# zhangmozhe/Deep-Exemplar-based-Video-Colorization

Hardware: AMD Instinct MI355X
Metric: colorized frames/sec/GPU at 216x384; correlation HBM GB/s vs roofline (higher is better)
Workload: dtype f32

## Files before the change

deep-exemplar-based-video-colorization_amd/dvc_amd/_lib.py:

```python
import ctypes
import os

_HERE = os.path.dirname(os.path.abspath(__file__))
DEBUG_BUILD = os.environ.get("DVC_DEBUG_LIB", "0") == "1"
LIB_PATH = os.path.join(_HERE, "libdvc_hip_debug.so" if DEBUG_BUILD else "libdvc_hip.so")
ABI_VERSION = 20

c_float_p = ctypes.c_void_p
c_i32 = ctypes.c_int32
c_i64 = ctypes.c_int64


class DvcConvDesc(ctypes.Structure):
    _fields_ = [
        ("N", c_i32), ("Cin", c_i32), ("H", c_i32), ("W", c_i32),
        ("Cout", c_i32), ("ksize", c_i32), ("stride", c_i32), ("dil", c_i32),
        ("pad", c_i32), ("pad_mode", c_i32), ("in_up", c_i32), ("in_sub", c_i32),
        ("act", c_i32), ("act_slope", ctypes.c_float), ("in_prelu", c_i32), ("cfg", c_i32), ("split_k", c_i32),
        ("x_batch_stride", c_i64), ("y_batch_stride", c_i64), ("res_batch_stride", c_i64),
        ("flags", c_i32), ("w_batch_stride", c_i64),
    ]


class DvcConvGroupItem(ctypes.Structure):
    _fields_ = [
        ("d", DvcConvDesc), ("x", ctypes.c_void_p), ("u_packed", ctypes.c_void_p), ("bias", ctypes.c_void_p),
        ("act_slope_ptr", ctypes.c_void_p), ("residual", ctypes.c_void_p), ("y", ctypes.c_void_p),
        ("workspace", ctypes.c_void_p), ("workspace_bytes", ctypes.c_size_t),
    ]


class DvcInstNormItem(ctypes.Structure):
    _fields_ = [
        ("x", ctypes.c_void_p), ("S", c_i32), ("bias", ctypes.c_void_p), ("act", c_i32), ("act_slope", ctypes.c_float),
        ("act_slope_ptr", ctypes.c_void_p), ("residual", ctypes.c_void_p), ("slope_ptr", ctypes.c_void_p),
        ("chan_scale", ctypes.c_void_p), ("eps", ctypes.c_float),
        ("N", c_i32), ("C", c_i32), ("H", c_i32), ("W", c_i32), ("up", c_i32), ("sub", c_i32), ("rpad", c_i32),
        ("x_batch_stride", c_i64), ("res_batch_stride", c_i64), ("y_batch_stride", c_i64), ("y", ctypes.c_void_p),
    ]


_VP = ctypes.c_void_p
SIGNATURES = {
    "dvc_abi_version": (ctypes.c_int, []),
    "dvc_last_error": (ctypes.c_char_p, []),
    "dvc_conv2d_out_hw": (ctypes.c_int, [ctypes.POINTER(DvcConvDesc), ctypes.POINTER(c_i32), ctypes.POINTER(c_i32)]),
    "dvc_conv2d": (ctypes.c_int, [ctypes.POINTER(DvcConvDesc), _VP, _VP, _VP, _VP, _VP, _VP, _VP, _VP, _VP, _VP,
                                  ctypes.c_size_t, _VP]),
    "dvc_winograd_weight_floats": (ctypes.c_size_t, [c_i32, c_i32]),
    "dvc_winograd_pack_weight": (ctypes.c_int, [_VP, c_i32, c_i32, _VP, _VP]),
    "dvc_conv2d_winograd_split": (ctypes.c_int, [ctypes.POINTER(DvcConvDesc), ctypes.c_size_t, ctypes.POINTER(c_i32),
                                                ctypes.POINTER(c_i32)]),
    "dvc_conv2d_winograd": (ctypes.c_int, [ctypes.POINTER(DvcConvDesc), _VP, _VP, _VP, _VP, _VP, _VP, _VP,
                                           ctypes.c_size_t, _VP]),
    "dvc_conv2d_winograd_pool": (ctypes.c_int, [ctypes.POINTER(DvcConvDesc), _VP, _VP, _VP, _VP, _VP, _VP, c_i64, _VP,
                                                ctypes.c_size_t, _VP]),
    "dvc_conv2d_winograd_dual": (ctypes.c_int, [ctypes.POINTER(DvcConvDesc), ctypes.POINTER(DvcConvDesc), _VP, _VP, _VP, _VP, _VP,
                                                _VP, _VP, ctypes.c_size_t, _VP]),
    "dvc_conv2d_ws_eligible": (ctypes.c_int, [ctypes.POINTER(DvcConvDesc)]),
    "dvc_conv2d_ws_pack_weight": (ctypes.c_int, [_VP, c_i32, c_i32, _VP, _VP]),
    "dvc_conv2d_ws": (ctypes.c_int, [ctypes.POINTER(DvcConvDesc), _VP, _VP, _VP, _VP, _VP, _VP]),
    "dvc_conv2d_winograd_group": (ctypes.c_int, [ctypes.POINTER(DvcConvGroupItem), c_i32, _VP]),
    "dvc_instnorm_apply_group": (ctypes.c_int, [ctypes.POINTER(DvcInstNormItem), c_i32, _VP]),
    "dvc_conv1x1_small": (ctypes.c_int, [_VP, _VP, _VP, c_i32, c_i32, c_i32, c_i32, c_i32, _VP, _VP]),
    "dvc_instnorm_stats": (ctypes.c_int, [_VP, c_i32, c_i32, c_i32, c_i64, ctypes.c_float, _VP, _VP, _VP, _VP]),
    "dvc_affine_act": (ctypes.c_int, [_VP, _VP, _VP, _VP, _VP, c_i32, c_i32, c_i32, c_i32, c_i32, c_i32,
                                      c_i64, c_i64, c_i64, _VP, _VP]),
    "dvc_instnorm_apply": (ctypes.c_int, [_VP, _VP, _VP, _VP, ctypes.c_float, c_i32, c_i32, c_i32, c_i32, c_i32,
                                          c_i32, c_i32, c_i64, c_i64, c_i64, _VP, _VP, _VP, _VP, c_i32, _VP, _VP]),
    "dvc_cx_prepare": (ctypes.c_int, [_VP, _VP, c_i32, c_i32, c_i32, c_i32, ctypes.c_float, _VP, _VP, _VP, _VP]),
    "dvc_cx_rows": (ctypes.c_int, [_VP, c_i32, c_i64, c_i64, c_i32, c_i32, ctypes.c_float, _VP, _VP, _VP, _VP, _VP, _VP]),
    "dvc_cx_colmax": (ctypes.c_int, [_VP, c_i32, c_i64, c_i64, _VP, _VP, c_i32, c_i32, c_i32, ctypes.c_float, _VP, _VP, _VP]),
    "dvc_cx_finish": (ctypes.c_int, [_VP, c_i32, c_i32, _VP, _VP, _VP]),
    "dvc_cx_rows_tq": (ctypes.c_int, [_VP, c_i32, c_i64, c_i64, c_i64, _VP, _VP, _VP, c_i32, c_i32, c_i32, ctypes.c_float, _VP, _VP,
                                      _VP]),
    "dvc_cx_ds": (ctypes.c_int, [_VP, c_i32, c_i64, c_i64, c_i64, _VP, _VP, _VP, _VP, _VP, _VP, _VP, _VP, _VP, ctypes.c_float, c_i32,
                                 c_i32, c_i32, c_i32, c_i32, ctypes.c_float, _VP, _VP, _VP]),
    "dvc_cx_normalize_bwd": (ctypes.c_int, [_VP, _VP, _VP, c_i32, c_i32, c_i32, ctypes.c_float, _VP, _VP]),
    "dvc_instnorm_apply_partials": (ctypes.c_int, [_VP, c_i32, _VP, c_i32, ctypes.c_float, _VP, _VP, _VP, _VP, ctypes.c_float,
                                                   c_i32, c_i32, c_i32, c_i32, c_i32, c_i32, c_i32, c_i64, c_i64, _VP, _VP, _VP,
                                                   _VP, c_i32, _VP, _VP]),
    "dvc_maxpool2x2": (ctypes.c_int, [_VP, c_i32, c_i32, c_i32, _VP, _VP]),
    "dvc_avgpool2x2": (ctypes.c_int, [_VP, c_i32, c_i32, c_i32, _VP, _VP]),
    "dvc_avgpool4x4": (ctypes.c_int, [_VP, c_i32, c_i32, c_i32, _VP, _VP]),
    "dvc_upsample_nearest": (ctypes.c_int, [_VP, c_i32, c_i32, c_i32, c_i32, _VP, _VP]),
    "dvc_channel_l2norm": (ctypes.c_int, [_VP, c_i32, c_i32, c_i32, ctypes.c_float, _VP, _VP]),
    "dvc_channel_l2norm_multi": (ctypes.c_int, [_VP, _VP, _VP, _VP, c_i32, c_i32, ctypes.c_float, _VP]),
    "dvc_gray2rgb": (ctypes.c_int, [_VP, c_i32, c_i32, c_i64, _VP, _VP]),
    "dvc_lab2rgb": (ctypes.c_int, [_VP, c_i32, c_i32, ctypes.c_float, _VP, _VP]),
    "dvc_pack_color_input": (ctypes.c_int, [_VP, c_i64, _VP, _VP, _VP, c_i64, _VP, c_i64, c_i32, c_i32, _VP, _VP]),
    "dvc_upsample_bilinear2x": (ctypes.c_int, [_VP, c_i32, c_i32, c_i32, ctypes.c_float, _VP, _VP]),
    "dvc_lum_guide_u8": (ctypes.c_int, [_VP, c_i64, _VP, _VP]),
    "dvc_fgs_workspace_bytes": (ctypes.c_size_t, [c_i32, c_i32, c_i32, c_i32, c_i32]),
    "dvc_fgs_filter": (ctypes.c_int, [_VP, _VP, c_i32, c_i32, c_i32, c_i32, ctypes.c_float, ctypes.c_float, c_i32,
                                      ctypes.c_float, _VP, _VP, ctypes.c_size_t, _VP]),
    "dvc_lab2rgb_u8": (ctypes.c_int, [_VP, _VP, c_i32, c_i32, _VP, _VP]),
    "dvc_rgb8_to_lab": (ctypes.c_int, [_VP, c_i32, c_i32, _VP, _VP]),
    "dvc_center_pad_workspace_bytes": (ctypes.c_size_t, [c_i32, c_i32]),
    "dvc_center_pad_is_fused": (ctypes.c_int, [c_i32, c_i32, c_i32, c_i32]),
    "dvc_center_pad": (ctypes.c_int, [_VP, c_i32, c_i32, c_i32, c_i32, _VP, _VP, ctypes.c_size_t, _VP]),
    "dvc_corr_prepare": (ctypes.c_int, [_VP, c_i32, c_i32, c_i32, ctypes.c_float, _VP, _VP, _VP]),
    "dvc_corr_workspace_bytes": (ctypes.c_size_t, [c_i32, c_i32]),
    "dvc_corr_fwd": (ctypes.c_int, [_VP, _VP, _VP, ctypes.c_float, ctypes.c_float, c_i32, c_i32, c_i32, c_i32,
                                    _VP, _VP, _VP, _VP, _VP, _VP, ctypes.c_size_t, _VP]),
    "dvc_corr_merge_pack": (ctypes.c_int, [_VP, ctypes.c_size_t, ctypes.c_float, c_i32, c_i32, _VP, _VP, _VP, _VP, _VP, _VP, _VP]),
    "dvc_corr_prepare_bf16": (ctypes.c_int, [_VP, c_i32, c_i32, c_i32, ctypes.c_float, _VP, _VP, _VP, _VP]),
    "dvc_corr_bf16_workspace_bytes": (ctypes.c_size_t, [c_i32, c_i32]),
    "dvc_corr_fwd_bf16": (ctypes.c_int, [_VP, _VP, _VP, _VP, _VP, ctypes.c_float, c_i32, c_i32, c_i32, c_i32,
                                         _VP, _VP, _VP, _VP, _VP, _VP, ctypes.c_size_t, _VP]),
    "dvc_corr_softmax_bwd": (ctypes.c_int, [_VP, _VP, _VP, _VP, _VP, _VP, _VP, ctypes.c_float, ctypes.c_float, c_i32, c_i32, c_i32, c_i64, c_i32,
                                            _VP, _VP, _VP, _VP]),
    "dvc_nlwa_workspace_bytes": (ctypes.c_size_t, [c_i32, c_i32, c_i32, c_i32, c_i32]),
    "dvc_nlwa_fwd": (ctypes.c_int, [_VP, c_i32, c_i32, c_i32, _VP, c_i32, c_i32, c_i32, c_i32, c_i32, c_i32, ctypes.c_float,
                                    ctypes.c_float, ctypes.c_float, ctypes.c_float, c_i32, ctypes.c_float, _VP, _VP,
                                    ctypes.c_size_t, _VP]),
    "dvc_lwa_fwd": (ctypes.c_int, [_VP, c_i32, c_i32, c_i32, _VP, c_i32, c_i32, c_i32, c_i32, c_i32, ctypes.c_float,
                                   ctypes.c_float, ctypes.c_float, c_i32, ctypes.c_float, _VP, _VP]),
    "dvc_lwa_bwd": (ctypes.c_int, [_VP, c_i32, c_i32, c_i32, _VP, c_i32, c_i32, c_i32, c_i32, c_i32, ctypes.c_float,
                                   ctypes.c_float, ctypes.c_float, c_i32, ctypes.c_float, _VP, _VP, _VP, _VP, _VP]),
    "dvc_flow_warp_bwd_workspace_bytes": (ctypes.c_size_t, [c_i32, c_i32, c_i32, c_i32]),
    "dvc_flow_warp_fwd": (ctypes.c_int, [_VP, _VP, c_i32, c_i32, c_i32, c_i32, c_i32, _VP, _VP]),
    "dvc_flow_warp_bwd": (ctypes.c_int, [_VP, _VP, _VP, c_i32, c_i32, c_i32, c_i32, c_i32, _VP, _VP, _VP, ctypes.c_size_t, _VP]),
    "dvc_bgemm_workspace_bytes": (ctypes.c_size_t, [c_i32, c_i32, c_i32, c_i32]),
    "dvc_bgemm": (ctypes.c_int, [_VP, _VP, _VP, c_i32, c_i32, c_i32, c_i32, c_i64, c_i64, c_i64, c_i64, c_i64, c_i64, c_i64, c_i64,
                                 c_i32, _VP]),
    "dvc_bgemm_splitk": (ctypes.c_int, [_VP, _VP, _VP, c_i32, c_i32, c_i32, c_i32, c_i64, c_i64, c_i64, c_i64, c_i64, c_i64, c_i64,
                                        c_i64, c_i32, _VP, ctypes.c_size_t, _VP]),
    "dvc_vgg_act_bwd": (ctypes.c_int, [_VP, _VP, _VP, c_i64, _VP, _VP]),
    "dvc_vgg_pool_act_bwd": (ctypes.c_int, [_VP, _VP, _VP, _VP, c_i32, c_i32, c_i32, c_i32, _VP, _VP]),
    "dvc_vgg_conv1_bwd": (ctypes.c_int, [_VP, _VP, c_i32, c_i32, c_i32, c_i32, _VP, _VP]),
    "dvc_lab2rgb_bwd": (ctypes.c_int, [_VP, c_i32, c_i32, ctypes.c_float, _VP, _VP, _VP]),
# ... 69 lines not shown
```

deep-exemplar-based-video-colorization_amd/dvc_amd/nets.py:

```python
import torch
import torch.nn as nn
from torch.autograd.function import once_differentiable

from . import arch, ops

_VGG_MEAN_BGR = (0.40760392, 0.45795686, 0.48501961)


_pack_epoch = 0


def pack_epoch():
    return _pack_epoch


class _PackCache:

    def __init__(self):
        self._d = {}

    def get(self, key, param, fn):
        params = param if isinstance(param, tuple) else (param,)
        tag = tuple((p.data_ptr(), _version_of(p), str(p.device)) for p in params)
        param = params[0]
# ... 329 lines not shown
        self.phi = nn.Conv2d(self.in_channels, self.inter_channels, kernel_size=1, stride=1, padding=0)
        self._cache = _PackCache()
        self.corr_precision = "fp32"

    def _use_bf16(self, temperature, WTA_scale_weight):
        return self.corr_precision == "bf16" and float(temperature) <= 1e-4 and WTA_scale_weight == 1

    def _pk(self, key, conv):
        return self._cache.get(key, conv.weight, ops.pack_conv_weight)

    def _conv3(self, key, conv, x, **kw):
        return ops.conv3x3(x, conv.weight, _packs(self._cache, key, conv.weight), conv.bias.detach(), layer="warp." + key, **kw)

    def prepare(self):
        for hd in arch.WARP_HEAD_PLAN:
            for ci in (hd.conv_a, hd.conv_b):
                _prepack(self._cache, f"{hd.name}.{ci}", getattr(self, hd.name)[ci])
        for b in range(arch.WARP_NUM_RESBLOCKS):
            _prepack(self._cache, f"layer.{b}.conv1", self.layer[b].conv1)
            _prepack(self._cache, f"layer.{b}.conv2", self.layer[b].conv2)
        self._pk("theta", self.theta)
        self._pk("phi", self.phi)

    def features(self, r2, r3, r4, r5):
        return self._trunk(self._heads(r2, r3, r4, r5))

    def _heads(self, r2, r3, r4, r5):
        feats = [r2, r3, r4, r5]
        N = r2.shape[0]
        h, w, rpad5 = arch.warp_trunk_geometry([x.shape[2:] for x in feats])
        trunk = torch.empty((N, arch.WARP_TRUNK_CH, h, w), device=r2.device, dtype=torch.float32)
        bs = arch.WARP_TRUNK_CH * h * w
        heads = arch.WARP_HEAD_PLAN
        seqs = [getattr(self, hd.name) for hd in heads]

        def conv_item(hd, ci, x, **kw):
            key, conv = f"{hd.name}.{ci}", seqs[hd.index][ci]
            return dict(x=x, weight=conv.weight, packs=_packs(self._cache, key, conv.weight), bias=conv.bias.detach(),
                        layer="warp." + key, pad_mode=ops.PAD_REFLECT, **kw)

        t1 = ops.conv3x3_group([conv_item(hd, hd.conv_a, feats[hd.index], defer_reduce=hd.stride_b == 1) for hd in heads])
        normed = ops.instnorm_apply_group([dict(x=t, out=None if isinstance(t, ops.ConvPartials) else t,
                                                slope_t=seq[hd.prelu_a].weight.detach()) for hd, seq, t in zip(heads, seqs, t1)])
        t2 = [None] * len(heads)
        for hd, seq in zip(heads, seqs):
            if hd.stride_b != 1:
                cb = seq[hd.conv_b]
                t2[hd.index] = ops.conv2d(normed[hd.index], self._pk(f"{hd.name}.{hd.conv_b}", cb), cb.bias.detach(),
                                          stride=hd.stride_b, pad_mode=ops.PAD_REFLECT, in_up=2 if hd.up_mid else 1)
        plain = [hd for hd in heads if hd.stride_b == 1]
        second = ops.conv3x3_group([conv_item(hd, hd.conv_b, normed[hd.index], in_up=2 if hd.up_mid else 1, defer_reduce=True)
                                    for hd in plain])
        for hd, t in zip(plain, second):
            t2[hd.index] = t
        ops.instnorm_apply_group([dict(x=t, slope_t=seq[hd.prelu_b].weight.detach(), up=2 if hd.up_out else 1,
                                       rpad=rpad5 if hd.name == "layer5_1" else 0,
                                       out=trunk[:, hd.index * arch.WARP_FEATURE_CH:(hd.index + 1) * arch.WARP_FEATURE_CH],
                                       out_batch_stride=bs) for hd, seq, t in zip(heads, seqs, t2)])
        return trunk

    def _trunk(self, x, saved=None):
        for b in range(arch.WARP_NUM_RESBLOCKS):
            blk = self.layer[b]
            a = blk.prelu.weight.detach()
            if saved is not None:
                planes = x.shape[0] * x.shape[1]
                r1, r2 = (torch.empty(planes, device=x.device, dtype=torch.float32) for _ in range(2))
                t = self._conv3(f"layer.{b}.conv1", blk.conv1, x, pad_mode=ops.PAD_REFLECT)
                n1 = ops.instnorm_apply(t, out=t, scale_out=r1)
                p1 = ops.warp_prelu_fwd(n1, a)
                t = self._conv3(f"layer.{b}.conv2", blk.conv2, p1, pad_mode=ops.PAD_REFLECT)
                n2 = ops.instnorm_apply(t, out=t, scale_out=r2)
                saved.update({f"x{b}": x, f"n1.{b}": n1, f"rstd1.{b}": r1, f"p1.{b}": p1, f"n2.{b}": n2, f"rstd2.{b}": r2})
                x = ops.warp_prelu_fwd(n2, a, skip=x)
                continue
            t = self._conv3(f"layer.{b}.conv1", blk.conv1, x, pad_mode=ops.PAD_REFLECT, defer_reduce=True)
            t = _norm_in_place(t, slope_t=a)
            t = self._conv3(f"layer.{b}.conv2", blk.conv2, t, pad_mode=ops.PAD_REFLECT, defer_reduce=True)
            x = _norm_in_place(t, residual=x, slope_t=a)
        return x

    def project(self, which, feats, bf16=False, saved=None):
        conv = getattr(self, which)
        t = ops.conv2d(feats, self._pk(which, conv), conv.bias.detach(), ksize=1, pad=0)
        if saved is not None:
            assert not bf16
            out, mean = ops.corr_prepare_with_mean(t)
            saved["t." + which], saved["mean." + which] = t, mean
            return out
        return ops.corr_prepare_bf16(t) if bf16 else ops.corr_prepare(t)

    _HEADS = tuple(arch.WARP_HEAD_ORDER)

    def _trunk_named_parameters(self):
        return [(n, p) for n, p in self.named_parameters() if n.split(".")[0] in ("layer", "theta", "phi")]

    def _head_named_parameters(self):
        return [(n, p) for n, p in self.named_parameters() if n.split(".")[0] in self._HEADS]

    def _takes_training_path(self):
        return self.training and torch.is_grad_enabled() and any(p.requires_grad for _, p in self._trunk_named_parameters())

    def _check_training_call(self, exemplar_cache, return_taps, defer_merge, detach_flag):
        unfrozen = [n for n, p in self._head_named_parameters() if p.requires_grad]
        if unfrozen:
            raise NotImplementedError(
                f"WarpNet: the training path gives the gradients of the residual trunk and the theta / phi projections only "
                f"(layer.*, theta.*, phi.*); {len(unfrozen)} head parameters require grad ({unfrozen[0]}, ...); freeze the heads: "
                "`for head in (net.layer2_1, net.layer3_1, net.layer4_1, net.layer5_1): "
                "[p.requires_grad_(False) for p in head.parameters()]`")
        for flag, what in ((exemplar_cache is not None, "exemplar_cache"), (return_taps, "return_taps"), (defer_merge, "defer_merge"),
                           (detach_flag, "detach_flag=True")):
            if flag:
                raise NotImplementedError(f"WarpNet: `{what}` is not supported on the training path (training mode, grad mode on, "
                                          "a trunk / projection parameter requiring grad); call under torch.no_grad() or .eval()")

    def _forward_with_grad(self, ins, temperature, WTA_scale_weight):
        B_lab_map, A2, A3, A4, A5, B2, B3, B4, B5 = ins
        fh, fw = int(B_lab_map.shape[2] / 4), int(B_lab_map.shape[3] / 4)
        _check_trainable(self._trunk_named_parameters(), "WarpNet")
        with torch.no_grad():
            trunkA = self._heads(A2, A3, A4, A5)
            trunkB = self._heads(B2, B3, B4, B5)
            blab = ops.avgpool4x4(B_lab_map)
        if (trunkA.shape[2], trunkA.shape[3]) != (fh, fw):
            raise RuntimeError(f"shape '[{B_lab_map.shape[0]}, 1, {fh}, {fw}]' is invalid for feature map "
                               f"of size {tuple(trunkA.shape[2:])}")
        return self._train_from_trunks(trunkA, trunkB, blab, temperature, WTA_scale_weight)

    def _train_from_trunks(self, trunkA, trunkB, blab, temperature, WTA_scale_weight=1):
        from .corr_autograd import fused_correlation
        N, _, fh, fw = trunkA.shape
        named = self._trunk_named_parameters()
        theta, phi = _WarpTrain.apply(trunkA, trunkB, self, tuple(n for n, _ in named), *(p for _, p in named))
        y, sim, _ = fused_correlation(theta, phi, blab.view(N, 3, -1), float(temperature), fh, fw, WTA_scale_weight)
        return _Up4.apply(y), _Up4.apply(sim)

    def _trunk_forward_saving(self, trunkA, trunkB, saved):
        N = trunkA.shape[0]
        F = self._trunk(torch.cat((trunkA, trunkB), 0), saved=saved)
        saved["F"] = F
        return self.project("theta", F[:N], saved=saved), self.project("phi", F[N:], saved=saved)

    def _trunk_backward(self, t, g_theta, g_phi, need, need_trunk_input_grad=False):
        grads = {}
        F = t["F"]
        M, C, h, w = F.shape
        N = M // 2
        dF = torch.empty_like(F)
        need_blocks = need_trunk_input_grad or any(n.startswith("layer.") for n in need)
        for which, g, sl in (("theta", g_theta, slice(0, N)), ("phi", g_phi, slice(N, M))):
            conv = getattr(self, which)
            dt = ops.warp_cn_bwd(t["t." + which], t["mean." + which], g.contiguous())
            if _wants(need, which):
                _put_wb(grads, need, which, *ops.warp_k1_wgrad(dt, F[sl]))
            if need_blocks:
                wt = self._cache.get("warp_bwd." + which, conv.weight,
                                     lambda w: ops.pack_conv_weight(w.detach().transpose(0, 1).contiguous()))
                ops.conv2d(dt.view(N, -1, h, w), wt, None, ksize=1, pad=0, out=dF[sl])
        if not need_blocks:
            return None, None, grads
        g = dF
        for b in reversed(range(arch.WARP_NUM_RESBLOCKS)):
            blk = self.layer[b]
            a = blk.prelu.weight.detach()
            c1, c2 = f"layer.{b}.conv1", f"layer.{b}.conv2"
            sp = torch.empty((2, M * C), device=F.device, dtype=torch.float64)
            dz, du, _ = ops.warp_norm_prelu_bwd(g, t[f"n2.{b}"], t[f"rstd2.{b}"], a, skip=t[f"x{b}"], slope_part=sp[0])
            if _wants(need, c2):
                _put_wb(grads, need, c2, *ops.cvn_wgrad(dz, ops.warp_reflect_pad(t[f"p1.{b}"])))
            wt, packs = _bwd_filters(self._cache, "warp_bwd." + c2, blk.conv2.weight, vgg_bwd_weight)
            gp = ops.conv3x3(dz, wt, packs, None, layer="warp_bwd." + c2)
            g = ops.warp_fold(gp)
            del gp, dz
            dz, _, _ = ops.warp_norm_prelu_bwd(g, t[f"n1.{b}"], t[f"rstd1.{b}"], a, slope_part=sp[1])
            if _wants(need, c1):
                _put_wb(grads, need, c1, *ops.cvn_wgrad(dz, ops.warp_reflect_pad(t[f"x{b}"])))
            if f"layer.{b}.prelu.weight" in need:
                grads[f"layer.{b}.prelu.weight"] = ops.warp_slope_sum(sp)
            if b == 0 and not need_trunk_input_grad:
                return None, None, grads
            wt, packs = _bwd_filters(self._cache, "warp_bwd." + c1, blk.conv1.weight, vgg_bwd_weight)
            gp = ops.conv3x3(dz, wt, packs, None, layer="warp_bwd." + c1)
            g = ops.warp_fold(gp, skip=du)
            del gp, dz, du
        return g[:N], g[N:], grads

    def _memo_exemplar_side(self, key_tensors, regime, compute):
        mode = ops.exemplar_memo_mode()
        if mode == "off":
            return compute()
        versions = [_version_of(t) for t in key_tensors]
        pfp = tuple((p.data_ptr(), _version_of(p)) for p in self.parameters())
        if any(v is None for v in versions) or any(v is None for _, v in pfp):
            return compute()
        fp = (pfp, regime, ops.conv_algo(), ops.direct_layers(), ops.fuse_reduce(), ops.autotune_enabled(),
              ops.batch_plan_enabled(), ops.group_heads(), ops.ws_conv_enabled())
        memo = getattr(self, "_exemplar_memo", None)
        if (memo is not None and memo[1] == fp and len(memo[0]) == len(key_tensors)
                and all(a is b and va == vb for (a, va), b, vb in zip(memo[0], key_tensors, versions))):
            if mode != "verify":
                return memo[2]
            fresh = compute()
            if _same_tensors(fresh, memo[2]):
                return memo[2]
            import warnings
            warnings.warn("DVC_EXEMPLAR_MEMO=verify: the memoised exemplar side differs from a recomputation although no key "
                          "tensor or WarpNet parameter changed identity or version — something wrote to them through `.data` "
                          "(unsupported with the memo on); using the recomputed value", RuntimeWarning, stacklevel=3)
            value = fresh
        else:
            value = compute()
        object.__setattr__(self, "_exemplar_memo", ([(t, v) for t, v in zip(key_tensors, versions)], fp, value))
        return value

    def __getstate__(self):
        state = dict(self.__dict__)
        state.pop("_exemplar_memo", None)
        return state

    def exemplar_side(self, B_lab_map, B2, B3, B4, B5, bf16=None):
        if bf16 is None:
            bf16 = self.corr_precision == "bf16"
        phi = self.project("phi", self.features(B2, B3, B4, B5), bf16=bf16)
        blab = ops.avgpool4x4(B_lab_map)
        return phi, blab

    def forward(self, B_lab_map, A_relu2_1, A_relu3_1, A_relu4_1, A_relu5_1, B_relu2_1, B_relu3_1,
                B_relu4_1, B_relu5_1, temperature=0.001 * 5, detach_flag=False, WTA_scale_weight=1,
                feature_noise=0, exemplar_cache=None, return_taps=False, defer_merge=False):
        ins = [B_lab_map, A_relu2_1, A_relu3_1, A_relu4_1, A_relu5_1, B_relu2_1, B_relu3_1, B_relu4_1,
               B_relu5_1]
        for t in ins:
            _check_input(t, "WarpNet")
        if self._takes_training_path():
            self._check_training_call(exemplar_cache, return_taps, defer_merge, detach_flag)
            return self._forward_with_grad([t.detach().contiguous().float() for t in ins], temperature, WTA_scale_weight)
        memo_key = (B_lab_map, B_relu2_1, B_relu3_1, B_relu4_1, B_relu5_1)
        ins = [t.detach().contiguous().float() for t in ins]
        B_lab_map, A2, A3, A4, A5, B2, B3, B4, B5 = ins
        image_height, image_width = B_lab_map.shape[2], B_lab_map.shape[3]
        fh, fw = int(image_height / 4), int(image_width / 4)
        A_features = self.features(A2, A3, A4, A5)
        if (A_features.shape[2], A_features.shape[3]) != (fh, fw):
            raise RuntimeError(f"shape '[{B_lab_map.shape[0]}, 1, {fh}, {fw}]' is invalid for feature map "
                               f"of size {tuple(A_features.shape[2:])}")
        bf16 = self._use_bf16(temperature, WTA_scale_weight)
        if exemplar_cache is not None:
            phi, blab = exemplar_cache
            if isinstance(phi, tuple) != bf16:
                raise RuntimeError("exemplar cache was built for a different corr_precision / temperature regime")
        else:
            phi, blab = self._memo_exemplar_side(memo_key, ("forward", bf16),
                                                 lambda: self.exemplar_side(B_lab_map, B2, B3, B4, B5, bf16=bf16))
        theta = self.project("theta", A_features, bf16=bf16)
        if bf16:
            res = ops.corr_fwd_bf16(theta, phi, blab.view(blab.shape[0], 3, -1), float(temperature), fh, fw,
                                    want_small=return_taps, want_argmax=return_taps)
        else:
            res = ops.corr_fwd(theta, phi, blab.view(blab.shape[0], 3, -1), float(temperature), fh, fw,
                               wta_scale=float(WTA_scale_weight), want_small=return_taps,
                               want_argmax=return_taps, defer_merge=defer_merge and not return_taps)
            if isinstance(res, ops.CorrPartials):
                return res, None
        if return_taps:
            return res["y_up"], res["sim_up"], dict(theta=theta, phi=phi, y_small=res["y_small"],
                                                    sim_small=res["sim_small"], argmax=res["argmax"],
                                                    A_features=A_features)
        return res["y_up"], res["sim_up"]


def cvn_bwd_weight(w, pad_to=None):
    wt = vgg_bwd_weight(w)
    if pad_to is not None and wt.shape[0] < pad_to:
        wt = torch.cat((wt, wt.new_zeros((pad_to - wt.shape[0],) + tuple(wt.shape[1:]))), dim=0).contiguous()
    return wt


class _CVNTrain(torch.autograd.Function):

# ... 236 lines not shown
```

deep-exemplar-based-video-colorization_amd/dvc_amd/ops.py:

```python
import ctypes
import os as _os
import sys
from typing import NamedTuple

import torch

from . import _lib
from ._lib import DvcConvDesc, DvcConvGroupItem, DvcInstNormItem

ACT_NONE, ACT_RELU, ACT_PRELU, ACT_LEAKY, ACT_TANH128 = 0, 1, 2, 3, 4
PAD_ZERO, PAD_REFLECT = 0, 1
EPS64 = sys.float_info.epsilon


def _p(t):
    return None if t is None else ctypes.c_void_p(t.data_ptr())


def _pv(t):
    return None if t is None else t.data_ptr()


_raw_stream = getattr(torch._C, "_cuda_getCurrentRawStream", None)
_raw_device = getattr(torch._C, "_cuda_getDevice", None)
# ... 48 lines not shown

    def __exit__(self, *exc):
        global _ws_scope
        _ws_scope = self.prev


def _workspace(device, nbytes, tag="corr"):
    if _ws_scope is not None:
        cache, key = _ws_scope, (tag, device.index)
    else:
        cache, key = _ws_cache, (tag, device.index, _stream_handle())
    ws = cache.get(key)
    if ws is None or ws.numel() < nbytes:
        ws = torch.empty(nbytes, device=device, dtype=torch.uint8)
        cache[key] = ws
    return ws


conv_record = None
layer_record = None


def _on_unless_0(v):
    return v != "0"


def _on_if_1(v):
    return v == "1"


def _memo_mode(v):
    return {"0": "off", "verify": "verify"}.get(v, "on")


def _layer_names(v):
    return None if v is None else frozenset(v.split(","))


class _Switch(NamedTuple):
    getter: str
    setter: str
    var: str
    env: str
    default: str
    parse: object
    launch: bool


_SWITCHES = (
    _Switch("autotune_enabled", None, "_autotune", "DVC_AUTOTUNE", "0", _on_if_1, True),
    _Switch("ws_conv_enabled", "set_ws_conv", "_ws_conv", "DVC_WS_CONV", "1", _on_unless_0, True),
    _Switch("pool_fusion", "set_pool_fusion", "_pool_fusion", "DVC_POOL_FUSION", "1", _on_unless_0, True),
    _Switch("dual_conv_enabled", "set_dual_conv", "_dual_conv", "DVC_DUAL_CONV", "1", _on_if_1, True),
    _Switch("fuse_reduce", "set_fuse_reduce", "_fuse_reduce", "DVC_FUSE_REDUCE", "1", _on_if_1, True),
    _Switch("conv_algo", None, "_conv_algo", "DVC_CONV_ALGO", "auto", str, True),
    _Switch("exemplar_memo_mode", None, "_exemplar_memo", "DVC_EXEMPLAR_MEMO", "1", _memo_mode, False),
    _Switch("gemm_lib", "set_gemm_lib", "_gemm_lib", "DVC_GEMM_LIB", "1", _on_unless_0, False),
    _Switch("gray_fusion", "set_gray_fusion", "_gray_fusion", "DVC_GRAY_FUSION", "1", _on_unless_0, True),
    _Switch("group_heads", "set_group_heads", "_group_heads", "DVC_GROUP_HEADS", "1", _on_unless_0, True),
    _Switch("fold_merge", "set_fold_merge", "_fold_merge", "DVC_FOLD_MERGE", "1", _on_if_1, True),
    _Switch("batch_plan_enabled", None, "_batch_plan", None, "0", _on_if_1, True),
    _Switch("direct_layers", None, "DEFAULT_DIRECT_LAYERS", "DVC_DIRECT_LAYERS", None, _layer_names, True),
)


def _flag_functions(var, getter, setter):
    g = globals()

    def get():
        return g[var]

    def set_(flag=True):
        g[var] = bool(flag)
    get.__name__ = get.__qualname__ = getter
    set_.__name__ = set_.__qualname__ = setter
    return get, set_


for _sw in _SWITCHES:
    globals()[_sw.var] = _sw.parse(_os.environ.get(_sw.env, _sw.default) if _sw.env else _sw.default)
    if _sw.setter:
        globals()[_sw.getter], globals()[_sw.setter] = _flag_functions(_sw.var, _sw.getter, _sw.setter)
del _sw


def launch_epoch():
    g = globals()
    return tuple(g[sw.getter]() for sw in _SWITCHES if sw.launch)


def autotune_enabled():
    return _autotune


def set_autotune(flag=True):
    global _autotune
    _autotune = bool(flag)
    if _autotune:
        _load_tuned()


def conv_algo():
    return _conv_algo


def set_conv_algo(algo):
    global _conv_algo
    if algo not in ("auto", "speed", "direct", "winograd"):
        raise ValueError("conv algo must be 'auto', 'speed', 'direct' or 'winograd'")
    _conv_algo = algo


def exemplar_memo_enabled():
    return _exemplar_memo != "off"


def exemplar_memo_mode():
    return _exemplar_memo


def set_exemplar_memo(flag=True):
    global _exemplar_memo
    _exemplar_memo = "verify" if flag == "verify" else ("on" if flag else "off")


_direct_layers = None


def direct_layers():
    if _direct_layers is not None:
        return _direct_layers
    if DEFAULT_DIRECT_LAYERS is not None:
        return DEFAULT_DIRECT_LAYERS
    from . import arch
    return arch.DIRECT_LAYERS


def set_direct_layers(names=None):
    global _direct_layers
    _direct_layers = None if names is None else frozenset(names)


DEFER_REDUCE = 1
BATCH_PLAN = 2
GRAY_INPUT = 4


class batch_plan:

    def __init__(self, on=True):
        self.on = bool(on)

    def __enter__(self):
        global _batch_plan
        self.prev, _batch_plan = _batch_plan, self.on
        return self

    def __exit__(self, *exc):
        global _batch_plan
        _batch_plan = self.prev


def batch_plan_enabled():
    return _batch_plan


# ... 104 lines not shown
    return (vh + 2 * pad - ext) // stride + 1, (vw + 2 * pad - ext) // stride + 1


def _conv_desc(N, Cin, H, W, Cout, *, ksize=3, stride=1, dil=1, pad=None, pad_mode=PAD_ZERO, in_up=1, in_sub=1, act=ACT_NONE,
               act_slope=0.0, in_prelu=False, cfg=-1, split_k=0, x_batch_stride=0, y_batch_stride=0, res_batch_stride=0, flags=0,
               w_batch_stride=0):
    return DvcConvDesc(N=N, Cin=Cin, H=H, W=W, Cout=Cout, ksize=ksize, stride=stride, dil=dil,
                       pad=dil * (ksize - 1) // 2 if pad is None else pad, pad_mode=pad_mode, in_up=in_up, in_sub=in_sub,
                       act=act, act_slope=float(act_slope), in_prelu=1 if in_prelu else 0, cfg=cfg, split_k=split_k,
                       x_batch_stride=x_batch_stride, y_batch_stride=y_batch_stride, res_batch_stride=res_batch_stride,
                       flags=flags, w_batch_stride=w_batch_stride)


def _record_conv(d, *, affine, in_prelu, residual, algo=None):
    rec = dict(N=d.N, Cin=d.Cin, H=d.H, W=d.W, Cout=d.Cout, ksize=d.ksize, stride=d.stride, dil=d.dil, pad=d.pad,
               pad_mode=d.pad_mode, in_up=d.in_up, in_sub=d.in_sub, affine=affine, in_prelu=in_prelu, residual=residual, act=d.act)
    if algo is not None:
        rec["algo"] = algo
    return rec


def record_layer(layer, Cin, Cout, H, W, *, dil=1, in_up=1, in_sub=1, eligible=True, **extra):
    layer_record.append(dict(layer=layer, Cin=Cin, Cout=Cout, H=H, W=W, dil=dil, in_up=in_up, in_sub=in_sub, eligible=eligible,
                             **extra))


def conv2d(x, w_packed, bias, *, ksize=3, stride=1, dil=1, pad=1, pad_mode=PAD_ZERO, in_up=1, in_sub=1,
           act=ACT_NONE, act_slope=0.0, act_slope_t=None, in_scale=None, in_shift=None, in_slope_t=None,
           residual=None, out=None, out_batch_stride=0, cfg=-1, split_k=0, tune=True, gray_input=False):
    lib = _lib.load()
    x_bs = 0
    if gray_input:
        assert x.dim() == 4 and x.shape[1] == 1 and w_packed.dim() == 3 and w_packed.shape[0] == 3 and cfg == -1 and split_k == 0, \
            (x.shape, w_packed.shape)
        if x.stride(3) != 1 or x.stride(2) != x.shape[3]:
            x = x.contiguous()
        x_bs = x.stride(0) if x.shape[0] > 1 else 0
        if not (isinstance(x, torch.Tensor) and x.is_cuda and x.dtype == torch.float32):
            raise RuntimeError("dvc_amd: `x` must be a float32 ROCm device tensor; no CPU fallback")
    _need_all(x=None if gray_input else x, w_packed=w_packed, bias=bias, in_scale=in_scale, in_shift=in_shift,
              in_slope=in_slope_t, act_slope=act_slope_t, residual=residual)
    N, Cin, H, W = x.shape
    if gray_input:
        Cin, tune = 3, False
    w_bs = 0
    if w_packed.dim() == 4:
        assert w_packed.shape[0] == N, (w_packed.shape, x.shape)
        w_bs = w_packed[0].numel() if N > 1 else 0
    wshape = tuple(w_packed.shape[-3:])
    assert wshape[0] == Cin and wshape[1] == ksize * ksize, (w_packed.shape, Cin, ksize)
    Cout = wshape[2]
    OH, OW = conv_out_hw(H, W, ksize, stride, dil, pad, in_up, in_sub)
    if out is None:
        out = torch.empty((N, Cout, OH, OW), device=x.device, dtype=torch.float32)
    d = _conv_desc(N, Cin, H, W, Cout, ksize=ksize, stride=stride, dil=dil, pad=pad, pad_mode=pad_mode, in_up=in_up,
                   in_sub=in_sub, act=act, act_slope=act_slope, in_prelu=in_slope_t is not None, cfg=cfg, split_k=split_k,
                   x_batch_stride=x_bs, y_batch_stride=out_batch_stride, flags=GRAY_INPUT if gray_input else 0,
                   w_batch_stride=w_bs)
    if residual is not None:
        assert tuple(residual.shape) == (N, Cout, OH, OW), (residual.shape, (N, Cout, OH, OW))
    if _autotune and tune and cfg == -1 and split_k == 0:
        key = (Cin, H, W, Cout, ksize, stride, dil, pad, pad_mode, in_up, in_sub, in_scale is not None,
               in_slope_t is not None, residual is not None, act, x.device.index, w_packed.dim() == 4)
        best = _tuned.get(key)
        if best is None:
            d1 = DvcConvDesc.from_buffer_copy(d)
            d1.N = 1
            best = _tune_conv(lib, d1, (x, w_packed, bias, in_scale, in_shift, in_slope_t, act_slope_t, residual, out))
            _tuned[key] = best
            _save_tuned()
        d.cfg, d.split_k = best
    if conv_record is not None:
        conv_record.append(_record_conv(d, affine=in_scale is not None, in_prelu=in_slope_t is not None,
                                        residual=residual is not None))
    ws = _workspace(x.device, CONV_WORKSPACE_BYTES, "conv")
    _bump_generation(ws)
    rc = lib.dvc_conv2d(ctypes.byref(d), _p(x), _p(w_packed), _p(bias), _p(in_scale), _p(in_shift),
                        _p(in_slope_t), _p(act_slope_t), _p(residual), _p(out),
                        ctypes.c_void_p(ws.data_ptr()), ws.numel(), _stream())
    _lib.check(rc, "dvc_conv2d")
    return out


def ws_eligible(Cin, Cout, dil=1, pad_mode=PAD_ZERO, in_up=1, in_sub=1, act=ACT_NONE):
    return (Cin in (32, 64, 128) and Cout % 64 == 0 and dil == 1 and pad_mode == PAD_ZERO and in_up == 1 and in_sub == 1
            and act in (ACT_NONE, ACT_RELU, ACT_PRELU, ACT_LEAKY))


def pack_ws_weight(w):
    lib = _lib.load()
    w = w.detach().contiguous().float()
    _need(w, "weight")
    Cout, Cin = w.shape[0], w.shape[1]
    u = torch.empty(Cout * Cin * 9, device=w.device, dtype=torch.float32)
    _lib.check(lib.dvc_conv2d_ws_pack_weight(_p(w), Cout, Cin, _p(u), _stream()), "dvc_conv2d_ws_pack_weight")
    return u


def conv2d_ws(x, u_packed, bias, Cout, *, act=ACT_NONE, act_slope=0.0, act_slope_t=None, out=None, out_batch_stride=0):
    lib = _lib.load()
    _need_all(x=x, u_packed=u_packed, bias=bias, act_slope=act_slope_t)
    N, Cin, H, W = x.shape
    assert u_packed.numel() == Cout * Cin * 9, (u_packed.shape, Cout, Cin)
    if out is None:
        out = torch.empty((N, Cout, H, W), device=x.device, dtype=torch.float32)
    d = _conv_desc(N, Cin, H, W, Cout, act=act, act_slope=act_slope, y_batch_stride=out_batch_stride)
    if conv_record is not None:
        conv_record.append(_record_conv(d, affine=False, in_prelu=False, residual=False, algo="direct-ws"))
    _lib.check(lib.dvc_conv2d_ws(ctypes.byref(d), _p(x), _p(u_packed), _p(bias), _p(act_slope_t), _p(out), _stream()), "dvc_conv2d_ws")
    return out


def pack_winograd_weight(w):
    lib = _lib.load()
    w = w.detach()
    _need(w, "weight")
    co, ci, kh, kw = w.shape
    assert (kh, kw) == (3, 3) and co % 32 == 0, w.shape
    u = torch.empty((co // 32, ci, 4, 32, 4), device=w.device, dtype=torch.float32)
    assert u.numel() == lib.dvc_winograd_weight_floats(co, ci)
    _lib.check(lib.dvc_winograd_pack_weight(_p(w), co, ci, _p(u), _stream()), "dvc_winograd_pack_weight")
    return u


def winograd_eligible(Cin, Cout, ksize=3, stride=1, dil=1, pad=1, in_affine=False, in_prelu=False):
    return (ksize == 3 and stride == 1 and dil in (1, 2) and pad == dil and not in_affine and not in_prelu
            and Cin % 8 == 0 and Cout % 64 == 0)


def winograd_selected(N, Cin, H, W, Cout, *, ksize=3, stride=1, dil=1, pad=1, in_up=1, in_sub=1, in_affine=False,
                      in_prelu=False, layer=None):
    if _conv_algo == "direct" or not winograd_eligible(Cin, Cout, ksize, stride, dil, pad, in_affine, in_prelu):
        return False
    if _conv_algo == "winograd":
        return True
    if _conv_algo == "auto" and layer is not None and layer in direct_layers():
        return False
    OH, OW = conv_out_hw(H, W, ksize, stride, dil, pad, in_up, in_sub)
    return _wino_rule(N, Cin, Cout, OH, OW, dil)


def _wino_rule(N, Cin, Cout, OH, OW, dil):
    return OH * OW >= 13 * 24


_conv_ws_generation = {}


def _bump_generation(ws):
    g = _conv_ws_generation.get(ws.data_ptr(), 0) + 1
    _conv_ws_generation[ws.data_ptr()] = g
    return g


class ConvPartials:

    def __init__(self, ws, S, shape, bias, act, act_slope, act_slope_t, generation, device, offset=0):
        self.ws, self.S, self.shape, self.bias = ws, S, tuple(shape), bias
        self.act, self.act_slope, self.act_slope_t, self.generation, self.device = act, act_slope, act_slope_t, generation, device
        self.offset = int(offset)

    def data_ptr(self):
        return self.ws.data_ptr() + self.offset

    def check_live(self):
        if self.generation != _conv_ws_generation.get(self.ws.data_ptr()):
# ... 811 lines not shown
```

include/dvc_hip.h:

```cpp
#ifndef DVC_HIP_H
#define DVC_HIP_H

#include <stddef.h>
#include <stdint.h>

#ifdef __cplusplus
extern "C" {
#endif

#pragma GCC visibility push(default)

typedef void* dvcStream;

#define DVC_ABI_VERSION 20

int dvc_abi_version(void);
const char* dvc_last_error(void);

enum { DVC_ACT_NONE = 0, DVC_ACT_RELU = 1, DVC_ACT_PRELU = 2, DVC_ACT_LEAKY = 3, DVC_ACT_TANH128 = 4 };
enum { DVC_PAD_ZERO = 0, DVC_PAD_REFLECT = 1 };

typedef struct DvcConvDesc {
    int32_t N, Cin, H, W;
    int32_t Cout;
    int32_t ksize;
    int32_t stride;
    int32_t dil;
    int32_t pad;
    int32_t pad_mode;
    int32_t in_up;
    int32_t in_sub;
    int32_t act;
    float   act_slope;
    int32_t in_prelu;
    int32_t cfg;
    int32_t split_k;
    int64_t x_batch_stride;
    int64_t y_batch_stride;
    int64_t res_batch_stride;
    int32_t flags;
    int64_t w_batch_stride;
} DvcConvDesc;
#define DVC_CONV_DEFER_REDUCE 1
#define DVC_CONV_BATCH_PLAN 2
#define DVC_CONV_GRAY_INPUT 4

int dvc_conv2d_out_hw(const DvcConvDesc* d, int32_t* OH, int32_t* OW);

int dvc_conv2d(const DvcConvDesc* d,
               const float* x, const float* w_packed, const float* bias ,
               const float* in_scale , const float* in_shift ,
               const float* in_slope_ptr ,
               const float* act_slope_ptr ,
               const float* residual , float* y,
               void* workspace , size_t workspace_bytes,
               dvcStream stream);

size_t dvc_winograd_weight_floats(int32_t Cout, int32_t Cin);
int dvc_winograd_pack_weight(const float* w, int32_t Cout, int32_t Cin, float* u_packed, dvcStream stream);
int dvc_conv2d_winograd_split(const DvcConvDesc* d, size_t workspace_bytes, int32_t* split, int32_t* images_per_launch);
int dvc_conv2d_winograd(const DvcConvDesc* d, const float* x, const float* u_packed,
                        const float* bias , const float* act_slope_ptr ,
                        const float* residual , float* y,
                        void* workspace , size_t workspace_bytes, dvcStream stream);
int dvc_conv2d_winograd_pool(const DvcConvDesc* d, const float* x, const float* u_packed, const float* bias ,
                             const float* act_slope_ptr , float* y , float* y_pool,
                             int64_t pool_batch_stride, void* workspace , size_t workspace_bytes, dvcStream stream);
int dvc_conv2d_winograd_dual(const DvcConvDesc* dA, const DvcConvDesc* dB, const float* xA, const float* xB,
                             const float* u_packed_cat, const float* bias ,
                             const float* act_slope_ptr , float* y,
                             void* workspace , size_t workspace_bytes, dvcStream stream);

int dvc_conv2d_ws_eligible(const DvcConvDesc* d);
int dvc_conv2d_ws_pack_weight(const float* w, int32_t Cout, int32_t Cin, float* u_packed, dvcStream stream);
int dvc_conv2d_ws(const DvcConvDesc* d, const float* x, const float* u_packed, const float* bias ,
                  const float* act_slope_ptr , float* y, dvcStream stream);

typedef struct DvcConvGroupItem {
    DvcConvDesc d;
    const float* x;
    const float* u_packed;
    const float* bias;
    const float* act_slope_ptr;
    const float* residual;
    float* y;
    void* workspace;
    size_t workspace_bytes;
} DvcConvGroupItem;
int dvc_conv2d_winograd_group(const DvcConvGroupItem* items, int32_t n_items, dvcStream stream);

int dvc_conv1x1_small(const float* x, const float* w, const float* bias, int32_t N, int32_t Cin,
                      int32_t HW, int32_t Cout, int32_t act, float* y, dvcStream stream);

int dvc_instnorm_stats(const float* x, int32_t N, int32_t C, int32_t HW, int64_t x_batch_stride,
                       float eps, const float* chan_scale, float* scale, float* shift,
                       dvcStream stream);

int dvc_affine_act(const float* x, const float* scale, const float* shift, const float* residual,
                   const float* slope_ptr, int32_t N, int32_t C, int32_t H, int32_t W, int32_t up,
                   int32_t rpad, int64_t x_batch_stride, int64_t res_batch_stride,
                   int64_t y_batch_stride, float* y, dvcStream stream);

int dvc_instnorm_apply(const float* x, const float* residual , const float* slope_ptr ,
                       const float* chan_scale , float eps, int32_t N, int32_t C, int32_t H,
                       int32_t W, int32_t up, int32_t sub, int32_t rpad, int64_t x_batch_stride,
                       int64_t res_batch_stride, int64_t y_batch_stride, float* y,
                       float* scale_out, float* shift_out,
                       const float* chan_scale2 , int32_t sub2, float* y2 ,
                       dvcStream stream);
int dvc_instnorm_apply_partials(const float* part, int32_t S, const float* bias, int32_t act, float act_slope,
                                const float* act_slope_ptr, const float* residual, const float* slope_ptr,
                                const float* chan_scale, float eps, int32_t N, int32_t C, int32_t H, int32_t W, int32_t up,
                                int32_t sub, int32_t rpad, int64_t res_batch_stride, int64_t y_batch_stride, float* y,
                                float* scale_out, float* shift_out, const float* chan_scale2, int32_t sub2, float* y2,
                                dvcStream stream);

typedef struct DvcInstNormItem {
    const float* x;
    int32_t S;
    const float* bias;
    int32_t act;
    float act_slope;
    const float* act_slope_ptr;
    const float* residual;
    const float* slope_ptr;
    const float* chan_scale;
    float eps;
    int32_t N, C, H, W, up, sub, rpad;
    int64_t x_batch_stride, res_batch_stride, y_batch_stride;
    float* y;
} DvcInstNormItem;
int dvc_instnorm_apply_group(const DvcInstNormItem* items, int32_t n_items, dvcStream stream);

int dvc_maxpool2x2(const float* x, int32_t planes, int32_t H, int32_t W, float* y, dvcStream stream);
int dvc_avgpool2x2(const float* x, int32_t planes, int32_t H, int32_t W, float* y, dvcStream stream);
int dvc_avgpool4x4(const float* x, int32_t planes, int32_t H, int32_t W, float* y, dvcStream stream);
int dvc_upsample_nearest(const float* x, int32_t planes, int32_t H, int32_t W, int32_t f, float* y,
                         dvcStream stream);
int dvc_channel_l2norm(const float* x, int32_t N, int32_t C, int32_t HW, float eps, float* y,
                       dvcStream stream);
// ... 144 lines not shown
```

Baseline: 439.8.

## Add dedicated MFMA kernel for 256-channel 1x1 projection convolutions

Adds a specialised HIP kernel for the 256->256 1x1 theta/phi projection. It uses fp32 MFMA 32x32x2 instructions with double-buffered LDS tiles filled by global_load_lds, and adds bias in the epilogue. It replaces the generic conv2d path when shapes match and autotune is off, aiming to cut the overhead of the general conv kernel for this GEMM-shaped op. It adds a new code path with a split-accumulation emulation, and a flag that enters the exemplar memo fingerprint.

New measurement: 440.3 (median of 5 runs). About the same (+0.1%).

```diff
diff --git a/deep-exemplar-based-video-colorization_amd/csrc/project.hip b/deep-exemplar-based-video-colorization_amd/csrc/project.hip
--- /dev/null
+++ b/deep-exemplar-based-video-colorization_amd/csrc/project.hip
@@ -0,0 +1,154 @@
+#include "common.h"
+
+#include <cstdint>
+
+namespace {
+
+typedef float f32x16 __attribute__((ext_vector_type(16)));
+#define PJ_AS1 __attribute__((address_space(1)))
+#define PJ_AS3 __attribute__((address_space(3)))
+
+constexpr int PJ_C = 256;
+constexpr int PJ_CK = 16;
+constexpr int PJ_KT = 32;
+constexpr int PJ_T = 64;
+constexpr int PJ_NCHUNK = PJ_C / PJ_CK;
+
+struct ProjArgs {
+    const float* x;
+    const float* w;
+    const float* bias;
+    float* y;
+    int P, tiles;
+    int S, cps;
+};
+
+__global__ __launch_bounds__(256) void project_k256_kernel(ProjArgs a) {
+    __shared__ __attribute__((aligned(16))) float s_x0[PJ_KT * PJ_T];
+    __shared__ __attribute__((aligned(16))) float s_x1[PJ_KT * PJ_T];
+    __shared__ __attribute__((aligned(16))) float s_w0[PJ_KT * PJ_T];
+    __shared__ __attribute__((aligned(16))) float s_w1[PJ_KT * PJ_T];
+
+    const int id = blockIdx.x, j = id >> 3;
+    const int tile = (j >> 2) * 8 + (id & 7);
+    if (tile >= a.tiles) return;
+    const int m0 = (j & 3) * PJ_T, p0 = tile * PJ_T;
+    const int n = blockIdx.y;
+    const int P = a.P;
+    const int tid = threadIdx.x;
+    const int lane = tid & 63, wave = __builtin_amdgcn_readfirstlane(tid >> 6);
+    const int l31 = lane & 31, hi = lane >> 5;
+    const int wm = wave >> 1, wn = wave & 1;
+    const float* xn = a.x + (long)n * PJ_C * P;
+
+    unsigned xofs[2], wofs[2];
+#pragma unroll
+    for (int i = 0; i < 2; ++i) {
+        const int q = tid + i * 256, row = q >> 4, c4 = (q & 15) * 4;
+        xofs[i] = (unsigned)(row * P + min(p0 + c4, P - 4));
+        wofs[i] = (unsigned)(row * PJ_C + m0 + c4);
+    }
+    auto issue = [&](int st, float* xs, float* ws) {
+        const float* xc = xn + (long)st * PJ_KT * P;
+        const float* wc = a.w + st * PJ_KT * PJ_C;
+#pragma unroll
+        for (int i = 0; i < 2; ++i) {
+            __builtin_amdgcn_global_load_lds((const PJ_AS1 void*)(xc + xofs[i]), (PJ_AS3 void*)(xs + (i * 256 + wave * 64) * 4), 16, 0, 0);
+            __builtin_amdgcn_global_load_lds((const PJ_AS1 void*)(wc + wofs[i]), (PJ_AS3 void*)(ws + (i * 256 + wave * 64) * 4), 16, 0, 0);
+        }
+    };
+
+    f32x16 out, tot, acc;
+#pragma unroll
+    for (int r = 0; r < 16; ++r) out[r] = tot[r] = 0.f;
+    const int aoff = hi * PJ_T + wm * 32 + l31, boff = hi * PJ_T + wn * 32 + l31;
+    const int S = a.S, cps = a.cps;
+
+    auto stage = [&](int st, const float* xs, const float* ws, float* xs_next, float* ws_next) {
+        if (st + 1 < PJ_C / PJ_KT) issue(st + 1, xs_next, ws_next);
+#pragma unroll
+        for (int c = 0; c < PJ_KT / PJ_CK; ++c) {
+#pragma unroll
+            for (int r = 0; r < 16; ++r) acc[r] = 0.f;
+#pragma unroll
+            for (int kk = 0; kk < PJ_CK; kk += 2) {
+                const float av = ws[(c * PJ_CK + kk) * PJ_T + aoff];
+                const float bv = xs[(c * PJ_CK + kk) * PJ_T + boff];
+                acc = __builtin_amdgcn_mfma_f32_32x32x2f32(av, bv, acc, 0, 0, 0);
+            }
+            tot += acc;
+            const int done = st * (PJ_KT / PJ_CK) + c + 1;
+            if (done % cps == 0 || done == PJ_NCHUNK) {
+                if (S == 1) out = tot;
+                else out += tot;
+#pragma unroll
+                for (int r = 0; r < 16; ++r) tot[r] = 0.f;
+            }
+        }
+        __syncthreads();
+    };
+
+    issue(0, s_x0, s_w0);
+    __syncthreads();
+    for (int st = 0; st < PJ_C / PJ_KT; st += 2) {
+        stage(st, s_x0, s_w0, s_x1, s_w1);
+        stage(st + 1, s_x1, s_w1, s_x0, s_w0);
+    }
+
+    const int p = p0 + wn * 32 + l31;
+    if (p >= P) return;
+    float* yn = a.y + (long)n * PJ_C * P + p;
+    const int co0 = m0 + wm * 32 + 4 * hi;
+    if (a.bias) {
+        float b[16];
+#pragma unroll
+        for (int r = 0; r < 16; ++r) b[r] = a.bias[co0 + (r & 3) + 8 * (r >> 2)];
+#pragma unroll
+        for (int r = 0; r < 16; ++r) out[r] += b[r];
+    }
+#pragma unroll
+    for (int r = 0; r < 16; ++r) yn[(long)(co0 + (r & 3) + 8 * (r >> 2)) * P] = out[r];
+}
+
+int pick_tw(int OW) {
+    int best = 32, best_w = cdiv(OW, 32) * 32;
+    for (int tw : {16, 8}) {
+        const int wpad = cdiv(OW, tw) * tw;
+        if (wpad < best_w) {
+            best = tw;
+            best_w = wpad;
+        }
+    }
+    return best;
+}
+int project_split(int H, int W) {
+    const int tw = pick_tw(W), ph = 2 * (32 / tw);
+    const long waves = 4L * cdiv(W, tw) * cdiv(H, ph) * (PJ_C / PJ_T);
+    int S = 1;
+    if (waves < 1536) {
+        S = (int)((2048 + waves - 1) / waves);
+        if (S > 4) S = 4;
+    }
+    return cdiv(PJ_NCHUNK, cdiv(PJ_NCHUNK, S));
+}
+
+}
+
+extern "C" int dvc_project_k256(const float* x, const float* w_packed, const float* bias, int32_t N, int32_t H, int32_t W, float* y,
+                                dvcStream stream) {
+    DVC_REQUIRE(x && w_packed && y, "dvc_project_k256: null argument");
+    DVC_REQUIRE(N > 0 && N <= 65535 && H > 0 && W > 0, "dvc_project_k256: bad shape (N %d H %d W %d)", N, H, W);
+    const long P = (long)H * W;
+    DVC_REQUIRE(P % 4 == 0 && P * PJ_C < (1L << 31), "dvc_project_k256: H * W must be a multiple of 4 and 256 * H * W < 2^31 (got %ld)", P);
+    DVC_REQUIRE(((reinterpret_cast<uintptr_t>(x) | reinterpret_cast<uintptr_t>(w_packed)) & 15) == 0,
+                "dvc_project_k256: x and w_packed must be 16-byte aligned");
+    ProjArgs a;
+    a.x = x; a.w = w_packed; a.bias = bias; a.y = y;
+    a.P = (int)P;
+    a.tiles = cdiv((int)P, PJ_T);
+    a.S = project_split(H, W);
+    a.cps = cdiv(PJ_NCHUNK, a.S);
+    hipLaunchKernelGGL(project_k256_kernel, dim3(cdiv(a.tiles, 8) * 8 * (PJ_C / PJ_T), N), dim3(256), 0, (hipStream_t)stream, a);
+    DVC_CHECK_LAUNCH("dvc_project_k256");
+    return 0;
+}
diff --git a/deep-exemplar-based-video-colorization_amd/dvc_amd/_lib.py b/deep-exemplar-based-video-colorization_amd/dvc_amd/_lib.py
--- a/deep-exemplar-based-video-colorization_amd/dvc_amd/_lib.py
+++ b/deep-exemplar-based-video-colorization_amd/dvc_amd/_lib.py
@@ -47,6 +47,7 @@
     "dvc_conv2d_out_hw": (ctypes.c_int, [ctypes.POINTER(DvcConvDesc), ctypes.POINTER(c_i32), ctypes.POINTER(c_i32)]),
     "dvc_conv2d": (ctypes.c_int, [ctypes.POINTER(DvcConvDesc), _VP, _VP, _VP, _VP, _VP, _VP, _VP, _VP, _VP, _VP,
                                   ctypes.c_size_t, _VP]),
+    "dvc_project_k256": (ctypes.c_int, [_VP, _VP, _VP, c_i32, c_i32, c_i32, _VP, _VP]),
     "dvc_winograd_weight_floats": (ctypes.c_size_t, [c_i32, c_i32]),
     "dvc_winograd_pack_weight": (ctypes.c_int, [_VP, c_i32, c_i32, _VP, _VP]),
     "dvc_conv2d_winograd_split": (ctypes.c_int, [ctypes.POINTER(DvcConvDesc), ctypes.c_size_t, ctypes.POINTER(c_i32),
diff --git a/deep-exemplar-based-video-colorization_amd/dvc_amd/nets.py b/deep-exemplar-based-video-colorization_amd/dvc_amd/nets.py
--- a/deep-exemplar-based-video-colorization_amd/dvc_amd/nets.py
+++ b/deep-exemplar-based-video-colorization_amd/dvc_amd/nets.py
@@ -435,7 +435,11 @@
 
     def project(self, which, feats, bf16=False, saved=None):
         conv = getattr(self, which)
-        t = ops.conv2d(feats, self._pk(which, conv), conv.bias.detach(), ksize=1, pad=0)
+        w = self._pk(which, conv)
+        if ops.project_k256_takes(feats, w):
+            t = ops.project_k256(feats, w, conv.bias.detach())
+        else:
+            t = ops.conv2d(feats, w, conv.bias.detach(), ksize=1, pad=0)
         if saved is not None:
             assert not bf16
             out, mean = ops.corr_prepare_with_mean(t)
@@ -548,7 +552,7 @@
         if any(v is None for v in versions) or any(v is None for _, v in pfp):
             return compute()
         fp = (pfp, regime, ops.conv_algo(), ops.direct_layers(), ops.fuse_reduce(), ops.autotune_enabled(),
-              ops.batch_plan_enabled(), ops.group_heads(), ops.ws_conv_enabled())
+              ops.batch_plan_enabled(), ops.group_heads(), ops.ws_conv_enabled(), ops.project_fused())
         memo = getattr(self, "_exemplar_memo", None)
         if (memo is not None and memo[1] == fp and len(memo[0]) == len(key_tensors)
                 and all(a is b and va == vb for (a, va), b, vb in zip(memo[0], key_tensors, versions))):
diff --git a/deep-exemplar-based-video-colorization_amd/dvc_amd/ops.py b/deep-exemplar-based-video-colorization_amd/dvc_amd/ops.py
--- a/deep-exemplar-based-video-colorization_amd/dvc_amd/ops.py
+++ b/deep-exemplar-based-video-colorization_amd/dvc_amd/ops.py
@@ -154,6 +154,18 @@
     if _sw.setter:
         globals()[_sw.getter], globals()[_sw.setter] = _flag_functions(_sw.var, _sw.getter, _sw.setter)
 del _sw
+
+
+_project_fused = _on_unless_0(_os.environ.get("DVC_PROJECT_FUSED", "1"))
+
+
+def project_fused():
+    return _project_fused
+
+
+def set_project_fused(flag=True):
+    global _project_fused
+    _project_fused = bool(flag)
 
 
 def launch_epoch():
@@ -424,6 +436,25 @@
     return out
 
 
+def project_k256_takes(x, w_packed):
+    return (_project_fused and not _autotune and x.dim() == 4 and tuple(w_packed.shape) == (256, 1, 256) and x.shape[1] == 256
+            and (x.shape[2] * x.shape[3]) % 4 == 0 and 0 < x.shape[2] * x.shape[3] < (1 << 23) and x.shape[0] <= 65535)
+
+
+def project_k256(x, w_packed, bias, out=None):
+    lib = _lib.load()
+    _need_all(x=x, w_packed=w_packed, bias=bias, out=out)
+    N, Cin, H, W = x.shape
+    assert Cin == 256 and tuple(w_packed.shape) == (256, 1, 256) and (bias is None or bias.numel() == 256), (x.shape, w_packed.shape)
+    if out is None:
+        out = torch.empty((N, 256, H, W), device=x.device, dtype=torch.float32)
+    assert tuple(out.shape) == (N, 256, H, W), out.shape
+    if conv_record is not None:
+        conv_record.append(_record_conv(_conv_desc(N, 256, H, W, 256, ksize=1, pad=0), affine=False, in_prelu=False, residual=False))
+    _lib.check(lib.dvc_project_k256(_p(x), _p(w_packed), _p(bias), N, H, W, _p(out), _stream()), "dvc_project_k256")
+    return out
+
+
 def ws_eligible(Cin, Cout, dil=1, pad_mode=PAD_ZERO, in_up=1, in_sub=1, act=ACT_NONE):
     return (Cin in (32, 64, 128) and Cout % 64 == 0 and dil == 1 and pad_mode == PAD_ZERO and in_up == 1 and in_sub == 1
             and act in (ACT_NONE, ACT_RELU, ACT_PRELU, ACT_LEAKY))
diff --git a/include/dvc_hip.h b/include/dvc_hip.h
--- a/include/dvc_hip.h
+++ b/include/dvc_hip.h
@@ -56,6 +56,9 @@
                void* workspace , size_t workspace_bytes,
                dvcStream stream);
 
+int dvc_project_k256(const float* x, const float* w_packed, const float* bias , int32_t N, int32_t H, int32_t W,
+                     float* y, dvcStream stream);
+
 size_t dvc_winograd_weight_floats(int32_t Cout, int32_t Cin);
 int dvc_winograd_pack_weight(const float* w, int32_t Cout, int32_t Cin, float* u_packed, dvcStream stream);
 int dvc_conv2d_winograd_split(const DvcConvDesc* d, size_t workspace_bytes, int32_t* split, int32_t* images_per_launch);
```
